# NVlabs/sionna

Hardware: NVIDIA H100
Metric: coded bits/s, LDPC5G n=8448 k=4224 BP-20 decode (higher is better)
Workload: dtype f32

## Files before the change

### sionna_b200/csrc/ldpc_bp_qc.cu

```cuda
#include <algorithm>
#include <climits>
#include <iterator>
#include <numeric>
#include <vector>
#include "sb_common.h"
#include "sb_math.h"
#include "sb_math2.cuh"
#include "ldpc_graph.h"
#include "ldpc_rules.cuh"

namespace {

constexpr int kLoop = INT_MAX;
constexpr int kRowMax[] = {kLoop, 20, 12, 8, 4};
constexpr int kColCut = 7, kColFused = 10;
constexpr int kColMax[] = {kLoop, 32, 20, 12, 8, 4, 2, kLoop, 12, 4, 1};
constexpr int kRowClasses = (int)std::size(kRowMax);
constexpr int kColClasses = (int)std::size(kColMax);

constexpr bool decreasing(const int* m, int lo, int hi) {
    for (int k = lo + 1; k < hi; ++k)
        if (m[k] >= m[k - 1]) return false;
    return true;
}
static_assert(decreasing(kRowMax, 0, kRowClasses), "row class bounds must decrease");
static_assert(decreasing(kColMax, 0, kColCut) && decreasing(kColMax, kColCut, kColFused), "column class bounds must decrease");
static_assert(kColFused == kColClasses - 1 && kColMax[kColFused] == 1, "the fused class holds degree-1 columns only");

constexpr int degree_class(const int* m, int lo, int hi, int d) {
    int k = hi - 1;
    while (k > lo && d > m[k]) --k;
    return k;
}

struct QcParams {
    int Z, n_rows, n_cols, nnz, N, E, E_alloc, n_in, n_out;
    int row_cls_end[kRowClasses];
    int col_cls_end[kColClasses];
    int row_cls_mod[kRowClasses];
    int col_cls_mod[kColClasses];
    const int4* row_info;
    const int4* col_info;
    const int2* col_edge;
    const int* in_idx;
    const int* out_pos;
    const int* slot_of_edge;
    const float* llr;
    float* out;
    float* state_out;
    long long B;
    int num_iter, hard_out, use_tma;
    int early;
    int* iters_out;
    const int2* row_edge;
    int tab_rep;
    float offset, llr_max;
};


#define SB_PHI_HI 16.635532f
#define SB_PHI_ZERO 14.7117348f
template <class LT, class Probe>
__device__ __forceinline__ uint2 phi_pass1_pair(unsigned b0, unsigned b1, float& P, const LT& lt, Probe probe) {
    const float a0 = __uint_as_float(b0 & 0x7fffffffu), a1 = __uint_as_float(b1 & 0x7fffffffu);
    const float2 p = sb_phif2(make_float2(a0, a1), lt);
    probe(a0, a1);
    P = __fadd_rn(P, p.x);
    P = __fadd_rn(P, p.y);
    return make_uint2(__float_as_uint(p.x) | (b0 & 0x80000000u), __float_as_uint(p.y) | (b1 & 0x80000000u));
}
template <class LT>
__device__ __forceinline__ unsigned phi_pass1(unsigned b0, float& P, const LT& lt) {
    const float p = sb_phif_s(__uint_as_float(b0 & 0x7fffffffu), lt);
    P = __fadd_rn(P, p);
    return __float_as_uint(p) | (b0 & 0x80000000u);
}
template <class LT>
__device__ __forceinline__ uint2 phi_pass2_pair(unsigned w0, unsigned w1, float P, unsigned par, float clip, const LT& lt) {
    const float2 m = fadd2(make_float2(__uint_as_float(w0 | 0x80000000u), __uint_as_float(w1 | 0x80000000u)),
                           make_float2(P, P));
    const float2 y = sb_phif2(m, lt);
    return make_uint2(__float_as_uint(fminf(y.x, clip)) | ((w0 ^ par) & 0x80000000u),
                      __float_as_uint(fminf(y.y, clip)) | ((w1 ^ par) & 0x80000000u));
}
template <class LT>
__device__ __forceinline__ unsigned phi_pass2(unsigned w0, float P, unsigned par, float clip, const LT& lt) {
    const float y = sb_phif_s(__fadd_rn(__uint_as_float(w0 | 0x80000000u), P), lt);
    return __float_as_uint(fminf(y, clip)) | ((w0 ^ par) & 0x80000000u);
}
__device__ __forceinline__ unsigned ldw(const float* q) { return __float_as_uint(*q); }
__device__ __forceinline__ void stw(float* q, unsigned w) { *q = __uint_as_float(w); }

template <class LT>
__device__ __noinline__ void cn_phi_qc(float* pm, int Z, int deg, float clip, int* sat_flag, LT lt) {
    const unsigned am = __activemask();
    float P = 0.f;
    unsigned par = 0;
    int l = 0;
#pragma unroll 2
    for (; l + 1 < deg; l += 2) {
        float* q0 = pm + l * Z;
        float* q1 = q0 + Z;
        const unsigned b0 = ldw(q0), b1 = ldw(q1);
        par ^= b0 ^ b1;
        const uint2 w = phi_pass1_pair(b0, b1, P, lt, [&](float a0, float a1) {
            if (l == 0 && __all_sync(am, a0 >= SB_PHI_HI && a1 >= SB_PHI_HI)) *sat_flag = 1;
        });
        stw(q0, w.x);
        stw(q1, w.y);
    }
    if (l < deg) {
        float* q0 = pm + l * Z;
        const unsigned b0 = ldw(q0);
        par ^= b0;
        stw(q0, phi_pass1(b0, P, lt));
    }
    par &= 0x80000000u;
    l = 0;
#pragma unroll 2
    for (; l + 1 < deg; l += 2) {
        float* q0 = pm + l * Z;
        float* q1 = q0 + Z;
        const uint2 y = phi_pass2_pair(ldw(q0), ldw(q1), P, par, clip, lt);
        stw(q0, y.x);
        stw(q1, y.y);
    }
    if (l < deg) stw(pm + l * Z, phi_pass2(ldw(pm + l * Z), P, par, clip, lt));
}

__device__ __forceinline__ unsigned vote_sign(unsigned S, int l, unsigned par) { return ((S >> l) << 31) ^ par; }

template <class LT>
__device__ __noinline__ void cn_vote_row(float* pm, int Z, int deg, unsigned U, unsigned S, float clip, LT lt) {
    const unsigned par = (unsigned)__popc(S) << 31;
    float P = 0.f;
    unsigned u = U;
    for (; u & (u - 1); u &= u - 1) {
        float* q0 = pm + (__ffs(u) - 1) * Z;
        u &= u - 1;
        float* q1 = pm + (__ffs(u) - 1) * Z;
        const uint2 w = phi_pass1_pair(ldw(q0), ldw(q1), P, lt, [](float, float) {});
        stw(q0, w.x);
        stw(q1, w.y);
    }
    if (u) {
        float* q0 = pm + (__ffs(u) - 1) * Z;
        stw(q0, phi_pass1(ldw(q0), P, lt));
    }
    const unsigned rest = ~U & (0xffffffffu >> (32 - deg));
    if (rest) {
        const unsigned y = __float_as_uint(fminf(sb_phif_s(P, lt), clip));
        for (unsigned r = rest; r; r &= r - 1) {
            const int l = __ffs(r) - 1;
            stw(pm + l * Z, y | vote_sign(S, l, par));
        }
    }
    for (u = U; u & (u - 1); u &= u - 1) {
        float* q0 = pm + (__ffs(u) - 1) * Z;
        u &= u - 1;
        float* q1 = pm + (__ffs(u) - 1) * Z;
        const uint2 y = phi_pass2_pair(ldw(q0), ldw(q1), P, par, clip, lt);
        stw(q0, y.x);
        stw(q1, y.y);
    }
    if (u) {
        float* q0 = pm + (__ffs(u) - 1) * Z;
        stw(q0, phi_pass2(ldw(q0), P, par, clip, lt));
    }
}

template <int D, class LT>
__device__ __forceinline__ void cn_phi_qc_reg(float* pm, int Z, float clip, int* sat_flag, const LT& lt) {
    const unsigned am = __activemask();
    unsigned w[D];
    float P = 0.f;
    unsigned par = 0;
#pragma unroll
    for (int l = 0; l + 1 < D; l += 2) {
        const unsigned b0 = ldw(pm + l * Z), b1 = ldw(pm + (l + 1) * Z);
        par ^= b0 ^ b1;
        const uint2 q = phi_pass1_pair(b0, b1, P, lt, [&](float a0, float a1) {
            if (l == 0 && __all_sync(am, a0 >= SB_PHI_HI && a1 >= SB_PHI_HI)) *sat_flag = 1;
        });
        w[l] = q.x;
        w[l + 1] = q.y;
    }
    if (D & 1) {
        const unsigned b0 = ldw(pm + (D - 1) * Z);
        par ^= b0;
        w[D - 1] = phi_pass1(b0, P, lt);
    }
    par &= 0x80000000u;
#pragma unroll
    for (int l = 0; l + 1 < D; l += 2) {
        const uint2 y = phi_pass2_pair(w[l], w[l + 1], P, par, clip, lt);
        stw(pm + l * Z, y.x);
        stw(pm + (l + 1) * Z, y.y);
    }
    if (D & 1) stw(pm + (D - 1) * Z, phi_pass2(w[D - 1], P, par, clip, lt));
}

template <class LT, int... DS>
__device__ __forceinline__ bool cn_phi_reg_of(float* pm, int Z, int deg, float clip, int* sat_flag, const LT& lt) {
    return ((deg == DS && (cn_phi_qc_reg<DS, LT>(pm, Z, clip, sat_flag, lt), true)) || ...);
}

template <int CLS, class LT>
__device__ __forceinline__ void cn_phi_dispatch(float* pm, int Z, int deg, float clip, int* sat_flag, const LT& lt) {
    if (CLS == 4 && cn_phi_reg_of<LT, 3, 4>(pm, Z, deg, clip, sat_flag, lt)) return;
    if (CLS == 3 && cn_phi_reg_of<LT, 5, 6, 7, 8>(pm, Z, deg, clip, sat_flag, lt)) return;
    cn_phi_qc<LT>(pm, Z, deg, clip, sat_flag, lt);
}

struct StrideEdges {
    float* pm;
    int Z;
    __device__ __forceinline__ float in(int l) const { return pm[l * Z]; }
    __device__ __forceinline__ void out(int l, float v) const { pm[l * Z] = v; }
    __device__ __forceinline__ float staged(int l) const { return pm[l * Z]; }
};

__device__ __forceinline__ float2 minsum_mags(float m1, float m2, int deg, float clip, float offset) {
    float min_e = (m2 == m1) ? m1 : __fadd_rn(__fsub_rn(m2, m1), m1);
    if (deg == 1) min_e = __fadd_rn(100000.f, m1);
    return make_float2(fminf(fmaxf(__fsub_rn(m1, offset), 0.f), clip), fminf(fmaxf(__fsub_rn(min_e, offset), 0.f), clip));
}
__device__ __forceinline__ float minsum_msg(float v, float m1, float2 o, unsigned par) {
    const float mag = (fabsf(v) == m1) ? o.y : o.x;
    return __uint_as_float(__float_as_uint(mag) | ((__float_as_uint(v) ^ par) & 0x80000000u));
}
template <int DMAX, bool EXACT>
__device__ __forceinline__ void cn_minsum_qc(float* pm, int Z, int deg, float clip, float offset) {
    float x[DMAX];
    float m1 = INFINITY, m2 = INFINITY;
    unsigned par = 0;
#pragma unroll
    for (int l = 0; l < DMAX; ++l) {
        float v = INFINITY;
        if (EXACT || l < deg) v = pm[l * Z];
        x[l] = v;
        float a = fabsf(v);
        m2 = fminf(m2, fmaxf(m1, a));
        m1 = fminf(m1, a);
        par ^= __float_as_uint(v);
    }
    par &= 0x80000000u;
    const float2 o = minsum_mags(m1, m2, deg, clip, offset);
#pragma unroll
    for (int l = 0; l < DMAX; ++l) {
        const float y = minsum_msg(x[l], m1, o, par);
        if (EXACT || l < deg) pm[l * Z] = y;
    }
}

__device__ __forceinline__ void cn_minsum_qc_loop(float* pm, int Z, int deg, float clip, float offset) {
    float m1 = INFINITY, m2 = INFINITY;
    unsigned par = 0;
    for (int l = 0; l < deg; ++l) {
        float v = pm[l * Z];
        float a = fabsf(v);
        m2 = fminf(m2, fmaxf(m1, a));
        m1 = fminf(m1, a);
        par ^= __float_as_uint(v);
    }
    par &= 0x80000000u;
    const float2 o = minsum_mags(m1, m2, deg, clip, offset);
    for (int l = 0; l < deg; ++l) pm[l * Z] = minsum_msg(pm[l * Z], m1, o, par);
}

template <int RULE, int CLS, class LT>
__device__ __forceinline__ void cn_qc(float* pm, int Z, int deg, float clip, float offset, int* sat_flag, const LT& lt) {
    if constexpr (RULE == SB_CN_BOXPLUS_PHI) {
        cn_phi_dispatch<CLS, LT>(pm, Z, deg, clip, sat_flag, lt);
    } else if constexpr (RULE == SB_CN_BOXPLUS) {
        cn_tanh(StrideEdges{pm, Z}, deg, clip);
    } else {
        constexpr int D = kRowMax[CLS];
        const float off = (RULE == SB_CN_MINSUM) ? 0.f : offset;
        if constexpr (D == kLoop) {
            cn_minsum_qc_loop(pm, Z, deg, clip, off);
        } else if constexpr (CLS == 4) {
            if (deg == 3) cn_minsum_qc<3, true>(pm, Z, deg, clip, off);
            else if (deg == 4) cn_minsum_qc<4, true>(pm, Z, deg, clip, off);
            else cn_minsum_qc<D, false>(pm, Z, deg, clip, off);
        } else if constexpr (CLS == 3) {
            if (deg == 5) cn_minsum_qc<5, true>(pm, Z, deg, clip, off);
            else if (deg == 6) cn_minsum_qc<6, true>(pm, Z, deg, clip, off);
            else if (deg == 7) cn_minsum_qc<7, true>(pm, Z, deg, clip, off);
            else cn_minsum_qc<D, true>(pm, Z, deg, clip, off);
        } else if constexpr (CLS == 2) {
            if (deg == 9) cn_minsum_qc<9, true>(pm, Z, deg, clip, off);
            else if (deg == 10) cn_minsum_qc<10, true>(pm, Z, deg, clip, off);
            else cn_minsum_qc<D, false>(pm, Z, deg, clip, off);
        } else {
            if (deg == 19) cn_minsum_qc<19, true>(pm, Z, deg, clip, off);
            else cn_minsum_qc<D, false>(pm, Z, deg, clip, off);
        }
    }
}

__device__ __forceinline__ float lds_f32(uint32_t a) {
    float v;
    asm volatile("ld.shared.f32 %0, [%1];" : "=f"(v) : "r"(a));
    return v;
}
__device__ __forceinline__ void sts_f32(uint32_t a, float v) {
    asm volatile("st.shared.f32 [%0], %1;" ::"r"(a), "f"(v) : "memory");
}
__device__ __forceinline__ int2 lds_i2(uint32_t a) {
    int2 v;
    asm volatile("ld.shared.v2.s32 {%0, %1}, [%2];" : "=r"(v.x), "=r"(v.y) : "r"(a));
    return v;
}

struct VnLane {
    uint32_t j4, j4w, jk;
};
__device__ __forceinline__ uint32_t vn_addr(int2 e, const VnLane& v) {
    return (uint32_t)e.x + (v.jk < (uint32_t)e.y ? v.j4w : v.j4);
}
__device__ __forceinline__ bool vn_in_row(int2 e, uint32_t addr, const VnLane& v) {
    return addr - (uint32_t)e.x - ((uint32_t)e.y >> 16) < ((uint32_t)e.y & 0xffffu);
}

template <int DMAX, bool CHECK, bool KEEPM, bool EXACT = false>
__device__ __forceinline__ float vn_qc(uint32_t ce_s, int deg, const VnLane& vl, float llr, float clip) {
    uint32_t addr[DMAX];
    float m[KEEPM ? DMAX : 1];
    bool on[DMAX];
    float acc = 0.f;
#pragma unroll
    for (int k = 0; k < DMAX; ++k) {
        int2 e = make_int2(0, 0);
        if (EXACT || k < deg) e = lds_i2(ce_s + 8 * k);
        addr[k] = vn_addr(e, vl);
        bool ok = EXACT || ((k < deg) && (!CHECK || vn_in_row(e, addr[k], vl)));
        on[k] = ok;
        float v = 0.f;
        if (ok) v = lds_f32(addr[k]);
        if (ok) acc = __fadd_rn(acc, v);
        if (KEEPM) m[KEEPM ? k : 0] = v;
    }
    float x_tot = __fadd_rn(acc, llr);
#pragma unroll
    for (int k = 0; k < DMAX; ++k) {
        float v = 0.f;
        if (KEEPM) v = m[KEEPM ? k : 0];
        else if (on[k]) v = lds_f32(addr[k]);
        float y = clipf(__fadd_rn(-v, x_tot), clip);
        if (on[k]) sts_f32(addr[k], y);
    }
    return x_tot;
}

template <int MODE>
__device__ __forceinline__ float vn_qc_loop(uint32_t ce_s, int deg, const VnLane& vl, float llr, float clip) {
    float acc = 0.f;
    if (MODE == 0)
        for (int k = 0; k < deg; ++k) {
            const int2 e = lds_i2(ce_s + 8 * k);
            const uint32_t a = vn_addr(e, vl);
            if (vn_in_row(e, a, vl)) acc = __fadd_rn(acc, lds_f32(a));
        }
    float x_tot = __fadd_rn(acc, llr);
    for (int k = 0; k < deg; ++k) {
        const int2 e = lds_i2(ce_s + 8 * k);
        const uint32_t a = vn_addr(e, vl);
        if (vn_in_row(e, a, vl))
            sts_f32(a, (MODE == 1) ? __fadd_rn(llr, 0.f) : clipf(__fadd_rn(-lds_f32(a), x_tot), clip));
    }
    return x_tot;
}

template <int CLS, bool EX>
__device__ __forceinline__ float vn_cls(uint32_t ce, int deg, const VnLane& vl, float llr, float clip) {
    constexpr int D = kColMax[CLS];
    if constexpr (D == kLoop) {
        return vn_qc_loop<0>(ce, deg, vl, llr, clip);
    } else if constexpr (CLS >= kColCut) {
        return vn_qc<D, true, true>(ce, deg, vl, llr, clip);
    } else if constexpr (D > 12) {
        if (CLS == 2 && EX && deg == 19) return vn_qc<19, false, true, true>(ce, deg, vl, llr, clip);
        if (CLS == 2 && EX && deg == 17) return vn_qc<17, false, true, true>(ce, deg, vl, llr, clip);
        return vn_qc<D, false, false>(ce, deg, vl, llr, clip);
    } else {
        if constexpr (CLS == 3) {
            if (EX && deg == 9) return vn_qc<9, false, true, true>(ce, deg, vl, llr, clip);
            if (EX && deg == 10) return vn_qc<10, false, true, true>(ce, deg, vl, llr, clip);
            if (EX && deg == 11) return vn_qc<11, false, true, true>(ce, deg, vl, llr, clip);
        } else if constexpr (CLS == 4) {
            if (EX && deg == 5) return vn_qc<5, false, true, true>(ce, deg, vl, llr, clip);
            if (EX && deg == 6) return vn_qc<6, false, true, true>(ce, deg, vl, llr, clip);
            if (EX && deg == 7) return vn_qc<7, false, true, true>(ce, deg, vl, llr, clip);
        } else if constexpr (CLS == 5) {
            if (EX && deg == 3) return vn_qc<3, false, true, true>(ce, deg, vl, llr, clip);
        } else {
            if (EX && deg == 1) return vn_qc<1, false, true, true>(ce, deg, vl, llr, clip);
        }
        return vn_qc<D, false, true, EX>(ce, deg, vl, llr, clip);
    }
}

struct WarpCtx {
    int G, grp, lane_i;
};

__device__ __forceinline__ int first_of(int start, int start_mod, const WarpCtx& w) {
    return start + (w.grp - start_mod + (w.grp < start_mod ? w.G : 0));
}

__device__ __forceinline__ void fused_vn(const QcParams& p, float* q, float c2v, int fw, int lane_i, const float* llr_s,
                                         float clip, unsigned char* hd) {
    int s = fw >> 16, vb = fw & 0xffff;
    int j = lane_i + s;
    j -= (j >= p.Z) ? p.Z : 0;
    float x_tot = __fadd_rn(__fadd_rn(0.f, c2v), llr_s[vb * p.Z + j]);
    *q = clipf(__fadd_rn(-c2v, x_tot), clip);
    if (hd) hd[vb * p.Z + j] = 0.f >= x_tot ? 1 : 0;
}

template <int RULE, int CLS, class LT>
__device__ __forceinline__ void cn_class(const QcParams& p, const WarpCtx& w, float* msg, const float* llr_s,
                                         const int4* s_row, int start, int end, float clip, bool fuse, int* sat_flag,
                                         const LT& lt, unsigned char* hd) {
    for (int rr = first_of(start, p.row_cls_mod[CLS], w); rr < end; rr += w.G) {
        int4 ri = s_row[rr];
        if (w.lane_i < ri.z) {
            float* pm = msg + ri.x * p.Z + w.lane_i;
            cn_qc<RULE, CLS, LT>(pm, p.Z, ri.y, clip, p.offset, sat_flag, lt);
            if (fuse && ri.w >= 0) {
                float* q = pm + (ri.y - 1) * p.Z;
                fused_vn(p, q, *q, ri.w, w.lane_i, llr_s, clip, hd);
            }
        }
    }
}

template <int RULE, class LT>
__device__ __forceinline__ void cn_all(const QcParams& p, const WarpCtx& w, float* msg, const float* llr_s,
                                       const int4* s_row, float clip, bool fuse, int* sat_flag, const LT& lt,
                                       unsigned char* hd) {
    const int* re = p.row_cls_end;
    cn_class<RULE, 0, LT>(p, w, msg, llr_s, s_row, 0, re[0], clip, fuse, sat_flag, lt, hd);
    cn_class<RULE, 1, LT>(p, w, msg, llr_s, s_row, re[0], re[1], clip, fuse, sat_flag, lt, hd);
    cn_class<RULE, 2, LT>(p, w, msg, llr_s, s_row, re[1], re[2], clip, fuse, sat_flag, lt, hd);
    cn_class<RULE, 3, LT>(p, w, msg, llr_s, s_row, re[2], re[3], clip, fuse, sat_flag, lt, hd);
    cn_class<RULE, 4, LT>(p, w, msg, llr_s, s_row, re[3], re[4], clip, fuse, sat_flag, lt, hd);
}

__device__ __forceinline__ unsigned unsat_bit31(unsigned b) {
    return __float_as_uint(__fadd_rn(fabsf(__uint_as_float(b)), -SB_PHI_ZERO));
}

template <class LT>
__device__ __forceinline__ void cn_vote_pass(const QcParams& p, const WarpCtx& w, float* msg, const float* llr_s,
                                             const int4* s_row, float clip, bool fuse, float phi_max, int* sat_flag,
                                             const LT& lt, unsigned char* hd) {
    const int Z = p.Z, Z4 = 4 * Z;
    const int msgb = (int)smem_u32(msg);
    const unsigned ylast = __float_as_uint(fminf(phi_max, clip));
    for (int rr = w.grp; rr < p.n_rows; rr += w.G) {
        const int4 ri = s_row[rr];
        const bool act = w.lane_i < ri.z;
        float c2v = 0.f;
        if (ri.y > 32) {
            if (act) {
                float* pm = msg + ri.x * Z + w.lane_i;
                cn_phi_qc<LT>(pm, Z, ri.y, clip, sat_flag, lt);
                c2v = pm[(ri.y - 1) * Z];
            }
        } else if (ri.y > 0) {
            const int deg = ri.y;
            const int a0 = msgb + 4 * (ri.x * Z + (act ? w.lane_i : 0));
            const int top = a0 + (deg - 1) * Z4;
            const unsigned last = __float_as_uint(lds_f32(top));
            unsigned own = unsat_bit31(last) >> 31, S = last >> 31;
            int a = top - Z4;
            if (!(deg & 1)) {
                const unsigned b = __float_as_uint(lds_f32(a));
                own = __funnelshift_l(unsat_bit31(b), own, 1);
                S = __funnelshift_l(b, S, 1);
                a -= Z4;
            }
            for (; a > a0; a -= 2 * Z4) {
                const unsigned b1 = __float_as_uint(lds_f32(a)), b0 = __float_as_uint(lds_f32(a - Z4));
                own = __funnelshift_l(unsat_bit31(b1), own, 1);
                own = __funnelshift_l(unsat_bit31(b0), own, 1);
                S = __funnelshift_l(b1, S, 1);
                S = __funnelshift_l(b0, S, 1);
            }
            const unsigned U = __reduce_or_sync(0xffffffffu, act ? own : 0u);
            if (!(U & ~(1u << (deg - 1)))) {
                float y = __uint_as_float(last & 0x7fffffffu);
#pragma unroll 1
                for (int k = 0; k < 2; ++k) y = sb_phif_s(y, lt);
                if (act) {
                    const unsigned yb = __float_as_uint(fminf(y, clip));
                    unsigned v = (S ^ (0u - (__popc(S) & 1u))) << (32 - deg);
                    const unsigned wl = ylast | (v & 0x80000000u);
                    sts_f32(top, __uint_as_float(wl));
                    c2v = __uint_as_float(wl);
                    int a = top - Z4;
                    if (!(deg & 1)) {
                        v <<= 1;
                        sts_f32(a, __uint_as_float(yb | (v & 0x80000000u)));
                        a -= Z4;
                    }
                    for (; a > a0; a -= 2 * Z4) {
                        sts_f32(a, __uint_as_float(yb | ((v << 1) & 0x80000000u)));
                        sts_f32(a - Z4, __uint_as_float(yb | ((v << 2) & 0x80000000u)));
                        v <<= 2;
                    }
                }
            } else if (act) {
                cn_vote_row<LT>(msg + ri.x * Z + w.lane_i, Z, deg, U, S, clip, lt);
                c2v = lds_f32(top);
            }
        }
        if (fuse && ri.w >= 0 && act)
            fused_vn(p, msg + (ri.x + ri.y - 1) * Z + w.lane_i, c2v, ri.w, w.lane_i, llr_s, clip, hd);
    }
}

__device__ __forceinline__ void syndrome_pass(const QcParams& p, const WarpCtx& w, const int4* s_row,
                                              const unsigned char* hd, int* unsat) {
    for (int rr = w.grp; rr < p.n_rows; rr += w.G) {
        const int4 ri = s_row[rr];
        if (w.lane_i < ri.z) {
            unsigned par = 0;
            for (int l = 0; l < ri.y; ++l) {
                const int2 e = __ldg(p.row_edge + ri.x + l);
                int j = w.lane_i + e.y;
                j -= (j >= p.Z) ? p.Z : 0;
                par ^= hd[e.x + j];
            }
            if (par) *unsat = 1;
        }
    }
}

template <int CLS, bool EX>
__device__ __forceinline__ void vn_class(const QcParams& p, const WarpCtx& w, const VnLane& vl, const float* llr_s,
                                         const int4* s_col, uint32_t s_ce, int start, int end, float clip,
                                         bool final_pass, long long b, unsigned char* hd) {
    for (int cc = first_of(start, p.col_cls_mod[CLS], w); cc < end; cc += w.G) {
        int4 ci = s_col[cc];
        if (w.lane_i < ci.z) {
            int v = ci.w + w.lane_i;
            float x_tot = vn_cls<CLS, EX>(s_ce + 8 * ci.x, ci.y, vl, llr_s[v], clip);
            if (hd) hd[v] = 0.f >= x_tot ? 1 : 0;
            if (final_pass) {
                int o = p.out_pos[v];
                if (o >= 0) {
                    x_tot = clipf(x_tot, clip);
                    p.out[(size_t)b * p.n_out + o] = decoder_out(x_tot, p.hard_out);
                }
            }
        }
    }
}

template <bool EX>
__device__ __forceinline__ void vn_all(const QcParams& p, const WarpCtx& w, const VnLane& vl, const float* llr_s,
                                       const int4* s_col, uint32_t s_ce, float clip, bool final_pass,
                                       bool with_fused, long long b, unsigned char* hd) {
    const int* ce = p.col_cls_end;
    vn_class<0, EX>(p, w, vl, llr_s, s_col, s_ce, 0, ce[0], clip, final_pass, b, hd);
    vn_class<1, EX>(p, w, vl, llr_s, s_col, s_ce, ce[0], ce[1], clip, final_pass, b, hd);
    vn_class<2, EX>(p, w, vl, llr_s, s_col, s_ce, ce[1], ce[2], clip, final_pass, b, hd);
    vn_class<3, EX>(p, w, vl, llr_s, s_col, s_ce, ce[2], ce[3], clip, final_pass, b, hd);
    vn_class<4, EX>(p, w, vl, llr_s, s_col, s_ce, ce[3], ce[4], clip, final_pass, b, hd);
    vn_class<5, EX>(p, w, vl, llr_s, s_col, s_ce, ce[4], ce[5], clip, final_pass, b, hd);
    vn_class<6, EX>(p, w, vl, llr_s, s_col, s_ce, ce[5], ce[6], clip, final_pass, b, hd);
    vn_class<7, EX>(p, w, vl, llr_s, s_col, s_ce, ce[6], ce[7], clip, final_pass, b, hd);
    vn_class<8, EX>(p, w, vl, llr_s, s_col, s_ce, ce[7], ce[8], clip, final_pass, b, hd);
    vn_class<9, EX>(p, w, vl, llr_s, s_col, s_ce, ce[8], ce[9], clip, final_pass, b, hd);
    if (with_fused) vn_class<10, EX>(p, w, vl, llr_s, s_col, s_ce, ce[9], ce[10], clip, final_pass, b, hd);
}

__device__ __forceinline__ void vn_init(const QcParams& p, const WarpCtx& w, const VnLane& vl, const float* llr_s,
                                        const int4* s_col, uint32_t s_ce) {
    for (int cc = w.grp; cc < p.n_cols; cc += w.G) {
        const int4 ci = s_col[cc];
        if (w.lane_i < ci.z) vn_qc_loop<1>(s_ce + 8 * ci.x, ci.y, vl, llr_s[ci.w + w.lane_i], 0.f);
    }
}

constexpr int kQcThreads = 768;

template <int RULE, int REP, bool EARLY>
__global__ void __launch_bounds__(kQcThreads, 1) ldpc_bp_qc_kernel(const __grid_constant__ QcParams p) {
    const int T = blockDim.x, tid = threadIdx.x, lane = tid & 31, warp = tid >> 5, W = T >> 5;
    const int Z = p.Z, N = p.N, Zb = (Z + 31) >> 5;
    unsigned char* const smem_raw = sb_smem + (RULE == SB_CN_BOXPLUS_PHI ? LogTab<REP>::bytes : 0);
    const int off_llr = p.E_alloc * 4;
    const int off_col = (off_llr + N * 4 + 15) & ~15;
    const int off_row = off_col + p.n_cols * 16;
    const int off_ce = off_row + p.n_rows * 16;
    const int off_bar = (off_ce + p.nnz * 8 + 15) & ~15;
    float* msg = reinterpret_cast<float*>(smem_raw);
    float* llr_s = reinterpret_cast<float*>(smem_raw + off_llr);
    int4* s_col = reinterpret_cast<int4*>(smem_raw + off_col);
    int4* s_row = reinterpret_cast<int4*>(smem_raw + off_row);
    int2* s_ce_p = reinterpret_cast<int2*>(smem_raw + off_ce);
    uint64_t* bar = reinterpret_cast<uint64_t*>(smem_raw + off_bar);
    int* sat_flag = reinterpret_cast<int*>(smem_raw + off_bar + 8);
    int* unsat = reinterpret_cast<int*>(smem_raw + off_bar + 12);
    unsigned char* hd = EARLY ? smem_raw + off_bar + 16 : nullptr;
    const uint32_t msgb = smem_u32(smem_raw);
    const uint32_t s_ce = msgb + off_ce;
    WarpCtx w;
    w.G = W / Zb;
    w.grp = warp / Zb;
    w.lane_i = (warp - w.grp * Zb) * 32 + lane;
    VnLane vl{4u * w.lane_i, 4u * (w.lane_i + Z), (4u * w.lane_i) << 16 | 0xffffu};
    asm("" : "+r"(vl.j4), "+r"(vl.j4w), "+r"(vl.jk));

    for (int i = tid; i < p.n_cols; i += T) s_col[i] = p.col_info[i];
    for (int i = tid; i < p.n_rows; i += T) s_row[i] = p.row_info[i];
    for (int i = tid; i < p.nnz; i += T) {
        const int2 e = p.col_edge[i];
        const uint32_t s4 = (uint32_t)e.y & 0xffffu;
        s_ce_p[i] = make_int2((int)(msgb + (uint32_t)e.x - s4), (int)(s4 << 16 | (uint32_t)e.y >> 16));
    }
    const LogTab<REP> lt(lane);
    if (RULE == SB_CN_BOXPLUS_PHI) LogTab<REP>::fill(tid, T);
    if (p.use_tma && tid == 0) mbar_init(bar);
    __syncthreads();

    const float clip = p.llr_max;
    const float phi_max = sb_phif(0.f);
    uint32_t tma_phase = 0;

    for (long long b = blockIdx.x; b < p.B; b += gridDim.x) {
        load_channel_llr(llr_s, p.llr + (size_t)b * p.n_in, p.in_idx, N, p.n_in, clip, p.use_tma, msg, bar, tma_phase,
                         tid, T);
        __syncthreads();
        if (tid == 0) *sat_flag = 0;
        vn_init(p, w, vl, llr_s, s_col, s_ce);
        __syncthreads();
        if (p.num_iter == 0) {
            for (int v = tid; v < N; v += T) {
                int o = p.out_pos[v];
                if (o >= 0) p.out[(size_t)b * p.n_out + o] = decoder_out(llr_s[v], p.hard_out);
            }
        }
        int limit = p.num_iter;
        for (int it = 0; it < limit; ++it) {
            if (EARLY && it > 0 && it < limit - 1) {
                if (tid == 0) *unsat = 0;
                __syncthreads();
                syndrome_pass(p, w, s_row, hd, unsat);
                __syncthreads();
                if (*unsat == 0) limit = it + 1;
            }
            const bool final_pass = it == limit - 1;
            const bool sc = *sat_flag != 0;
            if (final_pass && tid == 0 && p.use_tma && b + gridDim.x < p.B)
                asm volatile("cp.async.bulk.prefetch.L2.global [%0], %1;" ::"l"(p.llr + (size_t)(b + gridDim.x) * p.n_in),
                             "r"((uint32_t)p.n_in * 4u) : "memory");
            if constexpr (RULE == SB_CN_BOXPLUS_PHI) {
                if (sc) cn_vote_pass(p, w, msg, llr_s, s_row, clip, !final_pass, phi_max, sat_flag, lt, hd);
                else cn_all<RULE>(p, w, msg, llr_s, s_row, clip, !final_pass, sat_flag, lt, hd);
            } else {
                cn_all<RULE>(p, w, msg, llr_s, s_row, clip, !final_pass, sat_flag, lt, hd);
            }
            __syncthreads();
            vn_all<true>(p, w, vl, llr_s, s_col, s_ce, clip, final_pass, final_pass, b, hd);
            __syncthreads();
        }
        if (EARLY && p.iters_out && tid == 0) p.iters_out[b] = limit;
        if (p.state_out) {
            store_state(p.state_out + (size_t)b * p.E, msg, p.slot_of_edge, p.E, tid, T);
            __syncthreads();
        }
    }
}

size_t qc_smem_bytes(const sb_ldpc_graph* g, int tab_rep, int early = 0) {
    return (early ? (size_t)g->N + 16 : 0) + ((size_t)g->qc_nnz * g->qc_Z + g->N) * 4 + 16 + (size_t)g->qc_cols * 16 + (size_t)g->qc_rows * 16 +
           (size_t)g->qc_nnz * 8 + 16 + 16 + (size_t)tab_rep * SB_LOGTAB_N * 8;
}

int qc_ensure_uploaded(sb_ldpc_graph* g) {
    if (g->qc_uploaded) return SB_OK;
    int rc;
    if ((rc = sb_upload(&g->d_qc_row_info, g->qc_row_info))) return rc;
    if ((rc = sb_upload(&g->d_qc_col_info, g->qc_col_info))) return rc;
    if ((rc = sb_upload(&g->d_qc_col_edge, g->qc_col_edge))) return rc;
    if ((rc = sb_upload(&g->d_qc_in_idx, g->qc_in_idx))) return rc;
    if ((rc = sb_upload(&g->d_qc_out_pos, g->qc_out_pos))) return rc;
    if ((rc = sb_upload(&g->d_qc_slot_of_edge, g->qc_slot_of_edge))) return rc;
    if ((rc = sb_upload(&g->d_qc_row_edge, g->qc_row_edge))) return rc;
    g->qc_uploaded = true;
    return SB_OK;
}

template <int RULE, bool EARLY>
int launch_qc(const sb_ldpc_graph* g, const QcParams& p, int threads, size_t smem, cudaStream_t stream) {
    auto kern = ldpc_bp_qc_kernel<RULE, 16, EARLY>;
    if constexpr (RULE == SB_CN_BOXPLUS_PHI) {
        if (p.tab_rep == 8) kern = ldpc_bp_qc_kernel<RULE, 8, EARLY>;
        if (p.tab_rep == 1) kern = ldpc_bp_qc_kernel<RULE, 1, EARLY>;
    }
    return sb_launch_decoder(kern, p, g, threads, smem, LLONG_MAX, stream, "sb_ldpc_decode(qc)");
}

}

void sb_qc_free_device(sb_ldpc_graph* g) {
    if (!g->qc_uploaded) return;
    cudaFree(g->d_qc_row_info); cudaFree(g->d_qc_col_info); cudaFree(g->d_qc_col_edge); cudaFree(g->d_qc_in_idx);
    cudaFree(g->d_qc_out_pos); cudaFree(g->d_qc_slot_of_edge); cudaFree(g->d_qc_row_edge);
    g->qc_uploaded = false;
}

extern "C" int sb_ldpc_graph_set_qc(sb_ldpc_graph* g, int32_t Z, int32_t n_entries, const int32_t* base_row,
                                    const int32_t* base_col, const int32_t* shift) {
    SB_CHECK_ARG(g && Z > 0 && Z <= 16383 && n_entries > 0 && base_row && base_col && shift, "sb_ldpc_graph_set_qc: bad arguments");
    SB_CHECK_ARG((int)g->h_cn.size() == g->E, "sb_ldpc_graph_set_qc: handle holds no edge list");
    SB_CHECK_ARG(!g->ref_order, "sb_ldpc_graph_set_qc: the QC kernel sums in ascending neighbour order; graphs created with "
                                "sb_ldpc_graph_create_ordered stay on the generic kernel");
    const int C = g->C, N = g->N, E = g->E;
    const int n_rows = (C + Z - 1) / Z, n_cols = (N + Z - 1) / Z;
    auto zrow = [&](int r) { return std::min(Z, C - r * Z); };
    auto zcol = [&](int c) { return std::min(Z, N - c * Z); };
    struct Ent { int r, c, s; };
    std::vector<Ent> ents;
    for (int k = 0; k < n_entries; ++k) {
        if (base_row[k] < 0 || base_col[k] < 0 || shift[k] < 0) { sb_set_error("sb_ldpc_graph_set_qc: negative entry"); return SB_EINVAL; }
        if (base_row[k] >= n_rows || base_col[k] >= n_cols) continue;
        ents.push_back({base_row[k], base_col[k], shift[k] % Z});
    }
    std::vector<long long> keys(E);
    for (int e = 0; e < E; ++e) keys[e] = ((long long)g->h_cn[e] << 32) | (unsigned)g->h_vn[e];
    std::sort(keys.begin(), keys.end());
    long long total = 0;
    for (const Ent& en : ents)
        for (int i = 0; i < zrow(en.r); ++i) {
            int j = (i + en.s) % Z;
            long long key = ((long long)(en.r * Z + i) << 32) | (unsigned)(en.c * Z + j);
            if (j >= zcol(en.c) || !std::binary_search(keys.begin(), keys.end(), key)) {
                sb_set_error("sb_ldpc_graph_set_qc: base entry (%d,%d,%d) does not match the graph", en.r, en.c, en.s);
                return SB_EINVAL;
            }
            ++total;
        }
    if (total != E) { sb_set_error("sb_ldpc_graph_set_qc: %lld lifted edges != %d graph edges", total, E); return SB_EINVAL; }
    std::vector<int> rdeg(n_rows, 0), cdeg(n_cols, 0);
    for (const Ent& en : ents) { ++rdeg[en.r]; ++cdeg[en.c]; }
    std::vector<std::vector<Ent>> by_row(n_rows), by_col(n_cols);
    for (const Ent& en : ents) { by_row[en.r].push_back(en); by_col[en.c].push_back(en); }
    for (auto& v : by_row) std::sort(v.begin(), v.end(), [](const Ent& a, const Ent& b) { return a.c < b.c; });
    for (auto& v : by_col) std::sort(v.begin(), v.end(), [](const Ent& a, const Ent& b) { return a.r < b.r; });
    std::vector<int> fused_col_of_row(n_rows, -1);
    std::vector<char> col_fused(n_cols, 0);
    for (int r = 0; r < n_rows; ++r) {
        if (by_row[r].empty()) continue;
        const Ent& last = by_row[r].back();
        if (cdeg[last.c] == 1 && rdeg[r] >= 2 && last.c < 65536 && zcol(last.c) == zrow(r)) {
            fused_col_of_row[r] = last.c;
            col_fused[last.c] = 1;
        }
    }
    auto row_class = [&](int r) { return degree_class(kRowMax, 0, kRowClasses, rdeg[r]); };
    auto col_class = [&](int c) {
        if (col_fused[c]) return kColFused;
        bool check = false;
        for (const Ent& en : by_col[c]) check = check || zrow(en.r) < Z;
        return check ? degree_class(kColMax, kColCut, kColFused, cdeg[c]) : degree_class(kColMax, 0, kColCut, cdeg[c]);
    };
    std::vector<int> rorder(n_rows), corder(n_cols);
    std::iota(rorder.begin(), rorder.end(), 0);
    std::iota(corder.begin(), corder.end(), 0);
    std::stable_sort(rorder.begin(), rorder.end(), [&](int a, int b) {
        return row_class(a) != row_class(b) ? row_class(a) < row_class(b) : rdeg[a] > rdeg[b]; });
    std::stable_sort(corder.begin(), corder.end(), [&](int a, int b) {
        return col_class(a) != col_class(b) ? col_class(a) < col_class(b) : cdeg[a] > cdeg[b]; });
    {
        const int Zb_ = (Z + 31) / 32;
        const int G = std::max(1, (kQcThreads / 32) / Zb_);
        auto balance = [&](std::vector<int>& order, const std::vector<int>& deg, auto cls_of) {
            std::vector<long long> load(G, 0);
            size_t pos = 0;
            while (pos < order.size()) {
                size_t end = pos;
                const int c = cls_of(order[pos]);
                while (end < order.size() && cls_of(order[end]) == c) ++end;
                std::vector<int> items(order.begin() + pos, order.begin() + end);
                std::stable_sort(items.begin(), items.end(), [&](int a, int b) { return deg[a] > deg[b]; });
                size_t next = 0;
                for (size_t r0 = pos; r0 < end; r0 += G) {
                    const size_t r1 = std::min(end, r0 + (size_t)G);
                    std::vector<size_t> slots;
                    for (size_t q = r0; q < r1; ++q) slots.push_back(q);
                    std::stable_sort(slots.begin(), slots.end(), [&](size_t a, size_t b) { return load[a % G] < load[b % G]; });
                    for (size_t q : slots) {
                        order[q] = items[next++];
                        load[q % G] += deg[order[q]];
                    }
                }
                pos = end;
            }
        };
        balance(rorder, rdeg, row_class);
        balance(corder, cdeg, col_class);
    }
    std::vector<int> row_cls_end(kRowClasses, 0), col_cls_end(kColClasses, 0);
    for (int r = 0; r < n_rows; ++r) for (int k = row_class(r); k < kRowClasses; ++k) ++row_cls_end[k];
    for (int c = 0; c < n_cols; ++c) for (int k = col_class(c); k < kColClasses; ++k) ++col_cls_end[k];
    std::vector<int> be_of((size_t)n_rows * n_cols, -1);
    std::vector<int> row_info(4 * n_rows), row_edge;
    int be = 0;
    for (int rr = 0; rr < n_rows; ++rr) {
        int r = rorder[rr];
        row_info[4 * rr] = be;
        row_info[4 * rr + 1] = rdeg[r];
        row_info[4 * rr + 2] = zrow(r);
        row_info[4 * rr + 3] = fused_col_of_row[r] >= 0 ? (fused_col_of_row[r] | (by_row[r].back().s << 16)) : -1;
        for (const Ent& en : by_row[r]) {
            if (be_of[(size_t)en.r * n_cols + en.c] != -1) { sb_set_error("sb_ldpc_graph_set_qc: duplicate base entry"); return SB_EINVAL; }
            be_of[(size_t)en.r * n_cols + en.c] = be++;
            row_edge.push_back(en.c * Z);
            row_edge.push_back(en.s);
        }
    }
    const int nnz = be;
    std::vector<int> col_info(4 * n_cols), col_edge(2 * (size_t)nnz);
    int ce = 0;
    for (int cc = 0; cc < n_cols; ++cc) {
        int c = corder[cc];
        col_info[4 * cc] = ce;
        for (const Ent& en : by_col[c]) {
            col_edge[2 * ce] = be_of[(size_t)en.r * n_cols + en.c] * Z * 4;
            col_edge[2 * ce + 1] = (en.s * 4) | ((zrow(en.r) * 4) << 16);
            ++ce;
        }
        col_info[4 * cc + 1] = cdeg[c];
        col_info[4 * cc + 2] = zcol(c);
        col_info[4 * cc + 3] = c * Z;
    }
    std::vector<int> in_nat(N), out_nat(N), slot(E);
    for (int r = 0; r < N; ++r) { in_nat[g->vn_order[r]] = g->in_idx[r]; out_nat[g->vn_order[r]] = g->out_pos[r]; }
    for (int e = 0; e < E; ++e) {
        int r = g->h_cn[e] / Z, i = g->h_cn[e] % Z, c = g->h_vn[e] / Z;
        slot[e] = be_of[(size_t)r * n_cols + c] * Z + i;
    }
    sb_qc_free_device(g);
    g->qc = true; g->qc_Z = Z; g->qc_rows = n_rows; g->qc_cols = n_cols; g->qc_nnz = nnz;
    g->qc_max_row_deg = *std::max_element(rdeg.begin(), rdeg.end());
    g->qc_max_col_deg = *std::max_element(cdeg.begin(), cdeg.end());
    g->qc_row_info.swap(row_info); g->qc_col_info.swap(col_info); g->qc_col_edge.swap(col_edge);
    g->qc_row_cls_end = row_cls_end; g->qc_col_cls_end = col_cls_end;
    g->qc_in_idx.swap(in_nat); g->qc_out_pos.swap(out_nat); g->qc_slot_of_edge.swap(slot); g->qc_row_edge.swap(row_edge);
    return SB_OK;
}

namespace {
__global__ void debug_phi_kernel(const float* x, float* o1, float* o2, long long n) {
    LogTab<16>::fill(threadIdx.x, blockDim.x);
    __syncthreads();
    const LogTab<16> lt(threadIdx.x & 31);
    long long i = (long long)blockIdx.x * blockDim.x + threadIdx.x;
    if (2 * i + 1 < n) {
        float2 r = sb_phif2(make_float2(x[2 * i], x[2 * i + 1]), lt);
        o2[2 * i] = r.x; o2[2 * i + 1] = r.y;
        o1[2 * i] = sb_phif(x[2 * i]); o1[2 * i + 1] = sb_phif(x[2 * i + 1]);
    }
}
}
extern "C" int sb_debug_phi(const float* d_x, float* d_scalar, float* d_packed, int64_t n, void* stream) {
    if (n == 0) return SB_OK;
    SB_CHECK_ARG(d_x && d_scalar && d_packed && n >= 0 && n % 2 == 0, "sb_debug_phi: bad arguments");
    debug_phi_kernel<<<(unsigned)((n / 2 + 255) / 256), 256, LogTab<16>::bytes, (cudaStream_t)stream>>>(d_x, d_scalar,
                                                                                                         d_packed, n);
    SB_LAUNCH_CHECK();
    return SB_OK;
}

extern "C" int sb_ldpc_graph_is_qc(const sb_ldpc_graph* g) { return g && g->qc ? 1 : 0; }

int sb_qc_try_decode(sb_ldpc_graph* g, const float* d_llr, int64_t batch, int32_t num_iter, int32_t cn_rule,
                     int32_t vn_rule, float offset, float llr_max, int32_t hard_out, const float* d_state_in,
                     float* d_state_out, float* d_out, cudaStream_t stream, bool* handled, int32_t early, int32_t* d_iters) {
    *handled = false;
    if (!g->qc || !g->flooding || vn_rule != SB_VN_SUM || d_state_in || cn_rule > SB_CN_OFFSET_MINSUM) return SB_OK;
    int tab_rep = cn_rule == SB_CN_BOXPLUS_PHI ? 16 : 0;
    if (tab_rep && qc_smem_bytes(g, tab_rep, early) > (size_t)g->smem_optin) tab_rep = 8;
    if (tab_rep && qc_smem_bytes(g, tab_rep, early) > (size_t)g->smem_optin) tab_rep = 1;
    const size_t smem = qc_smem_bytes(g, tab_rep, early);
    if (smem > (size_t)g->smem_optin) return SB_OK;
    if ((cn_rule == SB_CN_MINSUM || cn_rule == SB_CN_OFFSET_MINSUM) &&
        !(llr_max < 100000.f && (float)(g->qc_max_row_deg - 1) * llr_max < 99000.f))
        return SB_OK;
    int rc = qc_ensure_uploaded(g);
    if (rc) return rc;
    QcParams p{};
    p.Z = g->qc_Z; p.n_rows = g->qc_rows; p.n_cols = g->qc_cols; p.nnz = g->qc_nnz; p.N = g->N; p.E = g->E;
    p.E_alloc = g->qc_nnz * g->qc_Z; p.n_in = g->n_in; p.n_out = g->n_out;
    for (int k = 0; k < kRowClasses; ++k) p.row_cls_end[k] = g->qc_row_cls_end[k];
    for (int k = 0; k < kColClasses; ++k) p.col_cls_end[k] = g->qc_col_cls_end[k];
    p.row_info = (const int4*)g->d_qc_row_info; p.col_info = (const int4*)g->d_qc_col_info;
    p.col_edge = (const int2*)g->d_qc_col_edge; p.in_idx = g->d_qc_in_idx; p.out_pos = g->d_qc_out_pos;
    p.slot_of_edge = g->d_qc_slot_of_edge;
    p.llr = d_llr; p.out = d_out; p.state_out = d_state_out; p.B = batch; p.num_iter = num_iter; p.hard_out = hard_out;
    p.offset = offset; p.llr_max = llr_max; p.tab_rep = tab_rep;
    p.early = early; p.iters_out = d_iters; p.row_edge = (const int2*)g->d_qc_row_edge;
    p.use_tma = (g->n_in % 4 == 0) && (g->n_in <= p.E_alloc) && ((reinterpret_cast<uintptr_t>(d_llr) & 15) == 0);
    const int Zb = (g->qc_Z + 31) / 32;
    const int max_warps = kQcThreads / 32;
    int groups = std::max(1, std::min(max_warps / Zb, std::max(g->qc_rows, g->qc_cols)));
    const int threads = groups * Zb * 32;
    for (int k = 0; k < kRowClasses; ++k) p.row_cls_mod[k] = (k ? g->qc_row_cls_end[k - 1] : 0) % groups;
    for (int k = 0; k < kColClasses; ++k) p.col_cls_mod[k] = (k ? g->qc_col_cls_end[k - 1] : 0) % groups;
    rc = sb_dispatch<SB_CN_BOXPLUS_PHI, SB_CN_OFFSET_MINSUM>(cn_rule, [&](auto R) {
        return p.early ? launch_qc<R, true>(g, p, threads, smem, stream) : launch_qc<R, false>(g, p, threads, smem, stream);
    });
    *handled = (rc == SB_OK);
    return rc;
}
```

### sionna_b200/csrc/ldpc_graph.h

```cpp
#pragma once
#include <stdint.h>
#include <algorithm>
#include <vector>
#include "sb_common.h"

struct sb_ldpc_graph {
    int C = 0, N = 0, E = 0, Lc = 0, Lv = 0, n_in = 0, n_out = 0, n_sub = 1, n_active = 0;
    bool flooding = true;
    bool ref_order = false;
    std::vector<int> cn_off, cn_cnt, vn_off, vn_cnt, in_idx, out_pos, slot_of_edge, sched, cn_order, vn_order;
    std::vector<uint32_t> vn_slot;
    std::vector<int> h_cn, h_vn;
    bool uploaded = false;
    int device = -1;
    int *d_cn_off = nullptr, *d_cn_cnt = nullptr, *d_vn_off = nullptr, *d_vn_cnt = nullptr, *d_in_idx = nullptr,
        *d_out_pos = nullptr, *d_slot_of_edge = nullptr, *d_sched = nullptr;
    uint16_t* d_vn_slot16 = nullptr;
    uint32_t* d_vn_slot32 = nullptr;
    int smem_optin = 0, num_sms = 0;
    bool qc = false;
    int qc_Z = 0, qc_rows = 0, qc_cols = 0, qc_nnz = 0, qc_max_row_deg = 0, qc_max_col_deg = 0;
    std::vector<int> qc_row_info;
    std::vector<int> qc_col_info;
    std::vector<int> qc_col_edge;
    std::vector<int> qc_in_idx, qc_out_pos, qc_slot_of_edge;
    std::vector<int> qc_row_edge;
    std::vector<int> qc_row_cls_end, qc_col_cls_end;
    int *d_qc_row_info = nullptr, *d_qc_col_info = nullptr, *d_qc_col_edge = nullptr, *d_qc_in_idx = nullptr,
        *d_qc_out_pos = nullptr, *d_qc_slot_of_edge = nullptr, *d_qc_row_edge = nullptr;
    bool qc_uploaded = false;
};

static const int kSmemOptinH100 = 232448;

int sb_qc_try_decode(sb_ldpc_graph* g, const float* d_llr, int64_t batch, int32_t num_iter, int32_t cn_rule,
                     int32_t vn_rule, float offset, float llr_max, int32_t hard_out, const float* d_state_in,
                     float* d_state_out, float* d_out, cudaStream_t stream, bool* handled, int32_t early = 0,
                     int32_t* d_iters = nullptr);
void sb_qc_free_device(sb_ldpc_graph* g);

template <typename T>
int sb_upload(T** d, const std::vector<T>& h) {
    SB_CUDA(cudaMalloc((void**)d, std::max<size_t>(1, h.size()) * sizeof(T)));
    if (h.size()) SB_CUDA(cudaMemcpy(*d, h.data(), h.size() * sizeof(T), cudaMemcpyHostToDevice));
    return SB_OK;
}

#if defined(__CUDACC__)
template <class Kernel, class Params>
int sb_launch_decoder(Kernel kern, const Params& p, const sb_ldpc_graph* g, int threads, size_t smem, long long max_grid,
                      cudaStream_t stream, const char* who) {
    SB_CUDA(cudaFuncSetAttribute(kern, cudaFuncAttributeMaxDynamicSharedMemorySize, (int)smem));
    int occ = 0;
    SB_CUDA(cudaOccupancyMaxActiveBlocksPerMultiprocessor(&occ, kern, threads, smem));
    if (occ < 1) { sb_set_error("%s: kernel does not fit (threads %d, smem %zu)", who, threads, smem); return SB_EUNSUPPORTED; }
    long long grid = std::min<long long>(p.B, std::min<long long>((long long)g->num_sms * occ, max_grid));
    kern<<<(unsigned)grid, threads, smem, stream>>>(p);
    SB_LAUNCH_CHECK();
    return SB_OK;
}

__device__ __forceinline__ float clipf(float x, float c) { return fminf(fmaxf(x, -c), c); }

__device__ __forceinline__ uint32_t smem_u32(const void* p) { return (uint32_t)__cvta_generic_to_shared(p); }
__device__ __forceinline__ void mbar_init(uint64_t* bar) {
    asm volatile("mbarrier.init.shared::cta.b64 [%0], %1;" ::"r"(smem_u32(bar)), "r"(1));
    asm volatile("fence.mbarrier_init.release.cluster;" ::: "memory");
}
__device__ __forceinline__ void mbar_expect_tx(uint64_t* bar, uint32_t bytes) {
    asm volatile("mbarrier.arrive.expect_tx.shared::cta.b64 _, [%0], %1;" ::"r"(smem_u32(bar)), "r"(bytes) : "memory");
}
__device__ __forceinline__ void mbar_wait(uint64_t* bar, uint32_t parity) {
    asm volatile(
        "{\n"
        ".reg .pred p;\n"
        "WAIT_%=:\n"
        "mbarrier.try_wait.parity.shared::cta.b64 p, [%0], %1;\n"
        "@p bra DONE_%=;\n"
        "bra WAIT_%=;\n"
        "DONE_%=:\n"
        "}\n" ::"r"(smem_u32(bar)), "r"(parity) : "memory");
}
__device__ __forceinline__ void tma_bulk_g2s(void* dst_smem, const void* src_gmem, uint32_t bytes, uint64_t* bar) {
    asm volatile("cp.async.bulk.shared::cluster.global.mbarrier::complete_tx::bytes [%0], [%1], %2, [%3];" ::"r"(
                     smem_u32(dst_smem)),
                 "l"(src_gmem), "r"(bytes), "r"(smem_u32(bar))
                 : "memory");
}

__device__ __forceinline__ float decoder_out(float x, int hard_out) {
    return hard_out ? (0.f >= x ? 1.f : 0.f) : __fmul_rn(x, -1.f);
}

__device__ __forceinline__ void load_channel_llr(float* llr_s, const float* row, const int* in_idx, int N, int n_in,
                                                 float clip, bool tma, float* stage, uint64_t* bar, uint32_t& phase,
                                                 int tid, int T) {
    if (tma) {
        if (tid == 0) {
            asm volatile("fence.proxy.async.shared::cta;" ::: "memory");
            mbar_expect_tx(bar, (uint32_t)n_in * 4u);
            tma_bulk_g2s(stage, row, (uint32_t)n_in * 4u, bar);
        }
        mbar_wait(bar, phase);
        phase ^= 1u;
        for (int v = tid; v < N; v += T) {
            int ii = in_idx[v];
            float l = ii >= 0 ? stage[ii] : (ii == -1 ? 0.f : -clip);
            llr_s[v] = __fmul_rn(clipf(l, clip), -1.f);
        }
    } else {
        for (int v = tid; v < N; v += T) {
            int ii = in_idx[v];
            float l = ii >= 0 ? __ldg(row + ii) : (ii == -1 ? 0.f : -clip);
            llr_s[v] = __fmul_rn(clipf(l, clip), -1.f);
        }
    }
}

__device__ __forceinline__ void store_state(float* st, const float* v2c, const int* slot_of_edge, int E, int tid, int T) {
    for (int e = tid; e < E; e += T) st[e] = __fmul_rn(v2c[slot_of_edge[e]], -1.f);
}

#endif
```

Measured before the change: 3.094 billion.

## Replace static grid-stride codeword loop with atomic dynamic work claiming

Persistent blocks now fetch their next codeword from a global atomic counter instead of striding by gridDim. One thread claims the next index during the final iteration and L2-prefetches its LLRs. This is meant to balance load when early termination makes per-codeword work uneven, and to narrow loop indices to int. It adds an atomic per codeword, a memset per launch, and a ring of counters.

```diff
diff --git a/sionna_b200/csrc/ldpc_bp_qc.cu b/sionna_b200/csrc/ldpc_bp_qc.cu
--- a/sionna_b200/csrc/ldpc_bp_qc.cu
+++ b/sionna_b200/csrc/ldpc_bp_qc.cu
@@ -55,6 +55,7 @@
     const int2* row_edge;
     int tab_rep;
     float offset, llr_max;
+    unsigned* next_cw;
 };
 
 
@@ -542,7 +543,7 @@
 template <int CLS, bool EX>
 __device__ __forceinline__ void vn_class(const QcParams& p, const WarpCtx& w, const VnLane& vl, const float* llr_s,
                                          const int4* s_col, uint32_t s_ce, int start, int end, float clip,
-                                         bool final_pass, long long b, unsigned char* hd) {
+                                         bool final_pass, int b, unsigned char* hd) {
     for (int cc = first_of(start, p.col_cls_mod[CLS], w); cc < end; cc += w.G) {
         int4 ci = s_col[cc];
         if (w.lane_i < ci.z) {
@@ -563,7 +564,7 @@
 template <bool EX>
 __device__ __forceinline__ void vn_all(const QcParams& p, const WarpCtx& w, const VnLane& vl, const float* llr_s,
                                        const int4* s_col, uint32_t s_ce, float clip, bool final_pass,
-                                       bool with_fused, long long b, unsigned char* hd) {
+                                       bool with_fused, int b, unsigned char* hd) {
     const int* ce = p.col_cls_end;
     vn_class<0, EX>(p, w, vl, llr_s, s_col, s_ce, 0, ce[0], clip, final_pass, b, hd);
     vn_class<1, EX>(p, w, vl, llr_s, s_col, s_ce, ce[0], ce[1], clip, final_pass, b, hd);
@@ -606,7 +607,8 @@
     uint64_t* bar = reinterpret_cast<uint64_t*>(smem_raw + off_bar);
     int* sat_flag = reinterpret_cast<int*>(smem_raw + off_bar + 8);
     int* unsat = reinterpret_cast<int*>(smem_raw + off_bar + 12);
-    unsigned char* hd = EARLY ? smem_raw + off_bar + 16 : nullptr;
+    int* next_b = sat_flag + 2;
+    unsigned char* hd = EARLY ? smem_raw + off_bar + 24 : nullptr;
     const uint32_t msgb = smem_u32(smem_raw);
     const uint32_t s_ce = msgb + off_ce;
     WarpCtx w;
@@ -632,7 +634,9 @@
     const float phi_max = sb_phif(0.f);
     uint32_t tma_phase = 0;
 
-    for (long long b = blockIdx.x; b < p.B; b += gridDim.x) {
+    const int claimer = T - 32;
+    const auto claim = [&]() { return (int)(gridDim.x + atomicAdd(p.next_cw, 1u)); };
+    for (int b = blockIdx.x; b < p.B; b = *next_b) {
         load_channel_llr(llr_s, p.llr + (size_t)b * p.n_in, p.in_idx, N, p.n_in, clip, p.use_tma, msg, bar, tma_phase,
                          tid, T);
         __syncthreads();
@@ -644,6 +648,8 @@
                 int o = p.out_pos[v];
                 if (o >= 0) p.out[(size_t)b * p.n_out + o] = decoder_out(llr_s[v], p.hard_out);
             }
+            if (tid == claimer) *next_b = claim();
+            __syncthreads();
         }
         int limit = p.num_iter;
         for (int it = 0; it < limit; ++it) {
@@ -656,9 +662,13 @@
             }
             const bool final_pass = it == limit - 1;
             const bool sc = *sat_flag != 0;
-            if (final_pass && tid == 0 && p.use_tma && b + gridDim.x < p.B)
-                asm volatile("cp.async.bulk.prefetch.L2.global [%0], %1;" ::"l"(p.llr + (size_t)(b + gridDim.x) * p.n_in),
-                             "r"((uint32_t)p.n_in * 4u) : "memory");
+            if (final_pass && tid == claimer) {
+                const int nb = claim();
+                *next_b = nb;
+                if (p.use_tma && nb < p.B)
+                    asm volatile("cp.async.bulk.prefetch.L2.global [%0], %1;" ::"l"(p.llr + (size_t)nb * p.n_in),
+                                 "r"((uint32_t)p.n_in * 4u) : "memory");
+            }
             if constexpr (RULE == SB_CN_BOXPLUS_PHI) {
                 if (sc) cn_vote_pass(p, w, msg, llr_s, s_row, clip, !final_pass, phi_max, sat_flag, lt, hd);
                 else cn_all<RULE>(p, w, msg, llr_s, s_row, clip, !final_pass, sat_flag, lt, hd);
@@ -681,6 +691,8 @@
     return (early ? (size_t)g->N + 16 : 0) + ((size_t)g->qc_nnz * g->qc_Z + g->N) * 4 + 16 + (size_t)g->qc_cols * 16 + (size_t)g->qc_rows * 16 +
            (size_t)g->qc_nnz * 8 + 16 + 16 + (size_t)tab_rep * SB_LOGTAB_N * 8;
 }
+
+constexpr int kNextRing = 256;
 
 int qc_ensure_uploaded(sb_ldpc_graph* g) {
     if (g->qc_uploaded) return SB_OK;
@@ -692,6 +704,7 @@
     if ((rc = sb_upload(&g->d_qc_out_pos, g->qc_out_pos))) return rc;
     if ((rc = sb_upload(&g->d_qc_slot_of_edge, g->qc_slot_of_edge))) return rc;
     if ((rc = sb_upload(&g->d_qc_row_edge, g->qc_row_edge))) return rc;
+    SB_CUDA(cudaMalloc((void**)&g->d_qc_next, kNextRing * sizeof(unsigned)));
     g->qc_uploaded = true;
     return SB_OK;
 }
@@ -711,7 +724,8 @@
 void sb_qc_free_device(sb_ldpc_graph* g) {
     if (!g->qc_uploaded) return;
     cudaFree(g->d_qc_row_info); cudaFree(g->d_qc_col_info); cudaFree(g->d_qc_col_edge); cudaFree(g->d_qc_in_idx);
-    cudaFree(g->d_qc_out_pos); cudaFree(g->d_qc_slot_of_edge); cudaFree(g->d_qc_row_edge);
+    cudaFree(g->d_qc_out_pos); cudaFree(g->d_qc_slot_of_edge); cudaFree(g->d_qc_row_edge); cudaFree(g->d_qc_next);
+    g->d_qc_next = nullptr;
     g->qc_uploaded = false;
 }
 
@@ -885,6 +899,7 @@
                      float* d_state_out, float* d_out, cudaStream_t stream, bool* handled, int32_t early, int32_t* d_iters) {
     *handled = false;
     if (!g->qc || !g->flooding || vn_rule != SB_VN_SUM || d_state_in || cn_rule > SB_CN_OFFSET_MINSUM) return SB_OK;
+    if (batch > INT_MAX - (1 << 20)) return SB_OK;
     int tab_rep = cn_rule == SB_CN_BOXPLUS_PHI ? 16 : 0;
     if (tab_rep && qc_smem_bytes(g, tab_rep, early) > (size_t)g->smem_optin) tab_rep = 8;
     if (tab_rep && qc_smem_bytes(g, tab_rep, early) > (size_t)g->smem_optin) tab_rep = 1;
@@ -913,6 +928,9 @@
     const int threads = groups * Zb * 32;
     for (int k = 0; k < kRowClasses; ++k) p.row_cls_mod[k] = (k ? g->qc_row_cls_end[k - 1] : 0) % groups;
     for (int k = 0; k < kColClasses; ++k) p.col_cls_mod[k] = (k ? g->qc_col_cls_end[k - 1] : 0) % groups;
+    const unsigned slot = __atomic_fetch_add(&g->qc_next_slot, 1u, __ATOMIC_RELAXED) % kNextRing;
+    p.next_cw = g->d_qc_next + slot;
+    SB_CUDA(cudaMemsetAsync(p.next_cw, 0, sizeof(unsigned), stream));
     rc = sb_dispatch<SB_CN_BOXPLUS_PHI, SB_CN_OFFSET_MINSUM>(cn_rule, [&](auto R) {
         return p.early ? launch_qc<R, true>(g, p, threads, smem, stream) : launch_qc<R, false>(g, p, threads, smem, stream);
     });
diff --git a/sionna_b200/csrc/ldpc_graph.h b/sionna_b200/csrc/ldpc_graph.h
--- a/sionna_b200/csrc/ldpc_graph.h
+++ b/sionna_b200/csrc/ldpc_graph.h
@@ -28,6 +28,8 @@
     std::vector<int> qc_row_cls_end, qc_col_cls_end;
     int *d_qc_row_info = nullptr, *d_qc_col_info = nullptr, *d_qc_col_edge = nullptr, *d_qc_in_idx = nullptr,
         *d_qc_out_pos = nullptr, *d_qc_slot_of_edge = nullptr, *d_qc_row_edge = nullptr;
+    unsigned* d_qc_next = nullptr;
+    unsigned qc_next_slot = 0;
     bool qc_uploaded = false;
 };
 
```

After: 3.122 billion (median of 6 runs). Within noise of the previous version (+0.9%).
